# ur-whitelab/nmrgnn

Measured on AMD Instinct MI355X. Metric: atoms/s (fwd+bwd) on 256-atom/16-neighbor synthetic graphs, higher is better.
Workload: dtype f32 (2xf16-piece MFMA, f32 accumulate)

## Files before the change

### include/nmrgnn_hip.h

```cpp
#ifndef NMRGNN_HIP_H
#define NMRGNN_HIP_H

#include <stdint.h>

#ifdef __cplusplus
extern "C" {
#endif

#define NG_ABI_VERSION 9

enum {
  NG_OK = 0,
  NG_ERR_INVALID = -1,
  NG_ERR_HIP = -2,
  NG_ERR_NOMEM = -3,
  NG_ERR_UNSUPPORTED = -4
};

enum { NG_ACT_NONE = 0, NG_ACT_SOFTPLUS = 1, NG_ACT_RELU = 2, NG_ACT_TANH = 3 };

typedef struct ng_ctx ng_ctx;

int ng_abi_version(void);
int ng_ctx_create(int device, ng_ctx** out);
// ... 88 lines not shown

int ng_mp_aggregate(ng_ctx*, void* stream, int64_t N, int K, int F, int E, const float* h,
                    const int32_t* nlist, const float* e, float* A);

int ng_mp_layer_fwd(ng_ctx*, void* stream, int64_t N, int K, int F, int E, int act, int residual,
                    const float* h, const int32_t* nlist, const float* e, const float* inv_degree,
                    const float* w, float* h_out, float* A_save, float* s_save);
int ng_mp_layer_wants_aggregate(int F, int E, int K);

int ng_mp_layer_bwd(ng_ctx*, void* stream, int64_t N, int K, int F, int E, int act,
                    const float* h, const int32_t* nlist, const float* e, const float* inv_degree,
                    const float* w, const float* A_save, const float* s_save,
                    const int32_t* csc_ptr, const int32_t* csc_edge, const float* dh_out,
                    float* dh_in, float* de, int de_accum, float* dw);

int ng_mp_edge_records(ng_ctx*, void* stream, int64_t N, int K, int E, const int32_t* csc_ptr,
                       const int32_t* csc_edge, const float* e, float* rec);
int ng_mp_layer_bwd_rec(ng_ctx*, void* stream, int64_t N, int K, int F, int E, int act,
                    const float* h, const int32_t* nlist, const float* e, const float* inv_degree,
                    const float* w, const float* A_save, const float* s_save,
                    const int32_t* csc_ptr, const int32_t* csc_edge, const float* dh_out,
                    float* dh_in, float* de, int de_accum, float* dw, const float* csc_rec);

int ng_mp_aggregate_csr(ng_ctx*, void* stream, int64_t N, int F, int E, const float* h,
                        const int32_t* row_ptr, const int32_t* col, const float* e, float* A);
int ng_mp_layer_fwd_csr(ng_ctx*, void* stream, int64_t N, int64_t nnz, int F, int E, int act, int residual,
                        const float* h, const int32_t* row_ptr, const int32_t* col, const float* e,
                        const float* inv_degree, const float* w, float* h_out, float* A_save, float* s_save);
int ng_mp_layer_bwd_csr(ng_ctx*, void* stream, int64_t N, int64_t nnz, int F, int E, int act, const float* h,
                        const int32_t* row_ptr, const int32_t* col, const int32_t* row_of, const float* e,
                        const float* inv_degree, const float* w, const float* A_save, const float* s_save,
                        const int32_t* csc_ptr, const int32_t* csc_edge, const float* dh_out, float* dh_in,
                        float* de, int de_accum, float* dw);

int ng_mp_layer_fwd_short(ng_ctx*, void* stream, int64_t N, int K, int F, int E, int act, int residual, const float* h,
                          const int32_t* nlist, const float* e, const float* inv_degree, const float* w, float* h_out);
int ng_mp_layer_fwd_short_csr(ng_ctx*, void* stream, int64_t N, int F, int E, int act, int residual, const float* h,
                              const int32_t* row_ptr, const int32_t* col, const float* e, const float* inv_degree,
                              const float* w, float* h_out);
int ng_mp_layer_short_ok(int64_t N, int K, int F, int E);
int ng_fc_head_ok(int64_t N, int F, int L, int C, int act);
int ng_fc_head_fwd(ng_ctx*, void* stream, int64_t N, int F, int L, int C, int act, const float* x,
                   const float* const* W, const float* const* b, const float* Wout, const float* bout,
                   const float* atoms, const float* pstd, const float* pavg, float* peaks);

int ng_build_incoming_lists(ng_ctx*, void* stream, int64_t N, int K, int64_t n_entries, const int32_t* nlist,
// ... 110 lines not shown
```

### nmrgnn_amd/_lib.py

```python
from __future__ import annotations

import ctypes as C
import os
import threading

_HERE = os.path.dirname(os.path.abspath(__file__))
LIB_PATH = os.environ.get("NMRGNN_HIP_LIB") or os.path.join(_HERE, "csrc", "libnmrgnn_hip.so")

NG_ACT_NONE, NG_ACT_SOFTPLUS, NG_ACT_RELU, NG_ACT_TANH = 0, 1, 2, 3
ACT_CODES = {None: NG_ACT_NONE, "linear": NG_ACT_NONE, "softplus": NG_ACT_SOFTPLUS, "relu": NG_ACT_RELU,
             "tanh": NG_ACT_TANH}

_c_float_p = C.POINTER(C.c_float)
_c_int32_p = C.POINTER(C.c_int32)
_vp = C.c_void_p
_i64 = C.c_int64
_u64 = C.c_uint64
_int = C.c_int
_f = C.c_float

SIGNATURES = {
    "ng_abi_version": (_int, []),
    "ng_ctx_create": (_int, [_int, C.POINTER(_vp)]),
    "ng_ctx_destroy": (None, [_vp]),
# ... 38 lines not shown
                                    C.POINTER(_vp), C.POINTER(_vp), _vp, _vp]),
    "ng_edge_mlp_bwd_live": (_int, [_vp, _vp, _i64, _int, _int, _int, _int, _vp, _vp, _vp, _vp, _vp, _f,
                                    C.POINTER(_vp), _vp, _vp, C.POINTER(_vp), C.POINTER(_vp), _int]),
    "ng_edge_mlp_dinput": (_int, [_vp, _vp, _i64, _int, _int, _int, _int, _vp, _vp, _vp, _vp, _vp, _f,
                                  C.POINTER(_vp), C.POINTER(_vp), _vp, _vp, _vp]),
    "ng_positions_grad": (_int, [_vp, _vp, _i64, _int, _vp, _vp, _vp, _vp, _f, _vp, _vp, _vp]),
    "ng_positions_grad_csr": (_int, [_vp, _vp, _i64, _i64, _vp, _vp, _vp, _vp, _vp, _f, _vp, _vp, _vp]),
    "ng_positions_grad_pbc": (_int, [_vp, _vp, _i64, _int, _vp, _vp, _vp, _vp, _f, _vp, _vp, _int, _vp, _int, _vp]),
    "ng_positions_grad_csr_pbc": (_int, [_vp, _vp, _i64, _i64, _vp, _vp, _vp, _vp, _vp, _f, _vp, _vp, _int, _vp, _int, _vp]),
    "ng_box_grad": (_int, [_vp, _vp, _i64, _int, _vp, _vp, _vp, _vp, _f, _int, _vp, _vp, _int, _vp, _vp]),
    "ng_box_grad_csr": (_int, [_vp, _vp, _i64, _i64, _vp, _vp, _vp, _vp, _f, _int, _vp, _vp, _int, _vp, _vp]),
    "ng_restraint_loss": (_int, [_vp, _vp, _int, _i64, _vp, _vp, _vp, _vp, _vp]),
    "ng_restraint_loss_ex": (_int, [_vp, _vp, _int, _i64, _int, _vp, _vp, _vp, _vp, _vp, _f, _vp, _vp, _vp, _vp]),
    "ng_embed_fwd": (_int, [_vp, _vp, _i64, _int, _int, _vp, _vp, _vp]),
    "ng_embed_bwd": (_int, [_vp, _vp, _i64, _int, _int, _vp, _vp, _vp]),
    "ng_mp_aggregate": (_int, [_vp, _vp, _i64, _int, _int, _int, _vp, _vp, _vp, _vp]),
    "ng_mp_layer_fwd": (_int, [_vp, _vp, _i64, _int, _int, _int, _int, _int, _vp, _vp, _vp, _vp, _vp,
                               _vp, _vp, _vp]),
    "ng_mp_layer_bwd": (_int, [_vp, _vp, _i64, _int, _int, _int, _int, _vp, _vp, _vp, _vp, _vp,
                               _vp, _vp, _vp, _vp, _vp, _vp, _vp, _int, _vp]),
    "ng_mp_layer_bwd_rec": (_int, [_vp, _vp, _i64, _int, _int, _int, _int, _vp, _vp, _vp, _vp, _vp,
                               _vp, _vp, _vp, _vp, _vp, _vp, _vp, _int, _vp, _vp]),
    "ng_mp_edge_records": (_int, [_vp, _vp, _i64, _int, _int, _vp, _vp, _vp, _vp]),
    "ng_mp_aggregate_csr": (_int, [_vp, _vp, _i64, _int, _int, _vp, _vp, _vp, _vp, _vp]),
    "ng_mp_layer_fwd_csr": (_int, [_vp, _vp, _i64, _i64, _int, _int, _int, _int, _vp, _vp, _vp, _vp, _vp, _vp,
                                   _vp, _vp, _vp]),
    "ng_mp_layer_bwd_csr": (_int, [_vp, _vp, _i64, _i64, _int, _int, _int, _vp, _vp, _vp, _vp, _vp, _vp, _vp,
                                   _vp, _vp, _vp, _vp, _vp, _vp, _vp, _int, _vp]),
    "ng_build_incoming_lists": (_int, [_vp, _vp, _i64, _int, _i64, _vp, _vp, _vp, _vp, _vp]),
    "ng_incoming_lists_scratch_bytes": (C.c_size_t, [_i64, _i64]),
    "ng_cutoff_count": (_int, [_vp, _vp, _int, _int, _f, _vp, _vp]),
    "ng_cutoff_fill": (_int, [_vp, _vp, _int, _int, _f, _f, _vp, _vp, _vp, _vp, _vp]),
    "ng_cutoff_fill_rows": (_int, [_vp, _vp, _int, _int, _f, _f, _vp, _vp, _vp, _vp, _vp, _vp]),
    "ng_cutoff_count_pbc": (_int, [_vp, _vp, _int, _int, _f, _vp, _vp, _int, _vp]),
    "ng_cutoff_fill_rows_pbc": (_int, [_vp, _vp, _int, _int, _f, _f, _vp, _vp, _int, _vp, _vp, _vp, _vp, _vp]),
    "ng_exclusive_scan_i32": (_int, [_vp, _vp, _i64, _vp, _vp]),
    "ng_dense_fwd": (_int, [_vp, _vp, _i64, _int, _int, _int, _int, _vp, _vp, _vp, _vp, _vp]),
    "ng_dense_bwd": (_int, [_vp, _vp, _i64, _int, _int, _int, _int, _vp, _vp, _vp, _vp, _vp, _vp,
                            _vp]),
    "ng_head_fwd": (_int, [_vp, _vp, _i64, _int, _int, _vp, _vp, _vp, _vp, _vp, _vp, _vp, _vp]),
    "ng_head_fwd_dropout": (_int, [_vp, _vp, _i64, _int, _int, _vp, _u64, _u64, _f, _vp, _vp, _vp, _vp, _vp, _vp, _vp]),
    "ng_head_bwd": (_int, [_vp, _vp, _i64, _int, _int, _vp, _vp, _vp, _vp, _vp, _vp, _vp, _vp, _vp]),
    "ng_head_loss_blocks": (_int, [_vp, _int, _int, _int, _i64]),
    "ng_head_loss_bwd": (_int, [_vp, _vp, _i64, _int, _int, _int, _i64, _vp, _u64, _u64, _f, _vp, _vp, _vp, _vp, _vp, _vp, _vp,
                               _vp, _vp, _f, _vp, _vp, _vp]),
    "ng_head_loss_reduce": (_int, [_vp, _vp, _vp, _int, _int, _int, _vp, _vp, _vp]),
# ... 128 lines not shown
```

### nmrgnn_amd/csrc/capi.hip

```cpp
#include <cmath>
#include <algorithm>
#include <cstring>
#include <map>
#include <new>

#include "ng_common.h"
#include "ng_internal.h"
#include "reduce.cuh"

namespace ng {

static Switches g_sw;
static bool g_sw_loaded = false;

static bool env_is(const char* name, const char* value) {
  const char* v = getenv(name);
  return v && !strcmp(v, value);
}

static void load_switches() {
  Switches s;
  s.edge_math_fp32 = env_is("NG_EDGE_MATH", "fp32");
  s.edge_bwd_math_fp32 = env_is("NG_EDGE_BWD_MATH", "fp32");
  s.gemm_math_fp32 = env_is("NG_GEMM_MATH", "fp32");
  s.edge_layered = env_is("NG_EDGE_PATH", "layered");
  s.mp_layered = env_is("NG_MP_PATH", "layered");
  s.fc_layered = env_is("NG_FC_PATH", "layered");
  s.dense_generic = env_is("NG_DENSE_PATH", "generic");
  s.head_generic = env_is("NG_HEAD_PATH", "generic");
  s.knn_serial = env_is("NG_KNN", "serial");
  s.knn_lanes = env_is("NG_KNN", "lanes");
  s.knn_cells = env_is("NG_KNN", "cells");
  s.knn_brute = env_is("NG_KNN", "brute");
  s.mp_gg_on = env_is("NG_MP_GG", "1");
  s.mp_gw_nowin = env_is("NG_MP_GW", "nowin");
  s.mp_w16 = !env_is("NG_MP_W16", "0");
  s.mp_wave = env_is("NG_MP_WAVE", "1") ? 1 : (env_is("NG_MP_WAVE", "0") ? 0 : -1);
  s.reduce_narrow = env_is("NG_REDUCE", "narrow");
  if (const char* v = getenv("NG_MP_GG_MIN_ROWS")) { const long long r = atoll(v); if (r >= 1) s.mp_gg_min_rows = r; }
  g_sw = s;
  g_sw_loaded = true;
}

const Switches& sw() {
  if (!g_sw_loaded) load_switches();
  return g_sw;
}

RangeGuard range_guard_begin(ng_ctx* ctx) {
  RangeGuard g;
  char* s = (char*)small_scratch(ctx);
  g.word = s ? reinterpret_cast<unsigned*>(s + NG_SMALL_BYTES - 64) : nullptr;
  if (++ctx->range_epoch == 0) ++ctx->range_epoch;
  g.epoch = ctx->range_epoch;
  return g;
}

const uint64_t* replay_state(ng_ctx* ctx) {
  if (!ctx->replay_armed) return nullptr;
  char* s = (char*)small_scratch(ctx);
// ... 445 lines not shown
```

### nmrgnn_amd/csrc/ng_common.h

```cpp
#pragma once
#include <hip/hip_runtime.h>

#include <cstdint>
#include <cstdio>
#include <string>
#include <map>
#include <utility>
#include <vector>

#include "../../include/nmrgnn_hip.h"

namespace ng {
struct RangeGuard {
  unsigned* word;
  unsigned epoch;
};

enum PackKind : int {
  PK_NONE = 0,
  PK_EDGE_H2 = 1,
  PK_EDGE_WT = 2,
  PK_EDGE_F32 = 3,
  PK_MPW_FWD = 4,
  PK_MPW_BWD = 5,
// ... 44 lines not shown
  uint64_t wjobs_hash = 0;
  std::vector<char> wjobs_host;
  uint32_t range_epoch = 0;
  void* comm = nullptr;
  int comm_rank = 0, comm_world = 1;
  bool defer_reduce = false;
  void* rq = nullptr;
  bool replay_armed = false;
  std::map<uint64_t, void*> wjobs_private;
  std::map<uint64_t, std::vector<WImage*>> wjobs_private_sel;
  uint64_t replay_token = 0;
};

namespace ng {

struct Switches {
  bool edge_math_fp32 = false, edge_bwd_math_fp32 = false, gemm_math_fp32 = false;
  bool edge_layered = false, mp_layered = false, fc_layered = false;
  bool dense_generic = false, head_generic = false, knn_serial = false, knn_cells = false, knn_brute = false;
  bool mp_gg_on = false;
  bool mp_gw_nowin = false;
  int mp_wave = -1;
  bool mp_w16 = true;
  bool reduce_narrow = false;
  bool knn_lanes = false;
  int64_t mp_gg_min_rows = 8192;
};
const Switches& sw();

struct DeviceGuard {
  int prev = -1;
  bool switched = false;
  explicit DeviceGuard(int dev) {
    if (hipGetDevice(&prev) == hipSuccess && prev != dev) switched = hipSetDevice(dev) == hipSuccess;
  }
  ~DeviceGuard() {
    if (switched) (void)hipSetDevice(prev);
  }
};

inline int fail(ng_ctx* ctx, int code, const std::string& msg) {
  if (ctx) ctx->err = msg;
  return code;
}

#define NG_HIP(ctx, expr)                                                              \
// ... 36 lines not shown
```

### nmrgnn_amd/engine.py

```python
from __future__ import annotations

import ctypes as C
import os

import numpy as np
import torch

from . import _lib
from ._lib import ptr, ptr_array
from .graph import GraphBatch
from .params import ParamStore

ACT = {None: 0, "linear": 0, "softplus": 1, "relu": 2, "tanh": 3}
DROPOUT_RATE = 0.2
FUSED_TAIL_MAX_ATOMS = 16384


def rbf_grid(low, high, count):
    lo, hi = np.float32(low), np.float32(high)
    delta = (hi - lo) / np.float32(count - 1)
    c = (lo + delta * np.arange(count, dtype=np.float32)).astype(np.float32)
    c[-1] = hi
    return c, float(np.float32(c[1] - c[0]))


def edge_path(edge_table, use_live_edges, live_kernels, E, n_edges, min_edges, is_csr, capturing):
    fits = n_edges * E * 4 < (1 << 31)
    sized = edge_table and E <= 8 and n_edges >= min_edges and fits
    if live_kernels and fits:
        return "table" if sized else ("live" if use_live_edges else "slots")
    if sized and not is_csr and not capturing:
        return "table_host"
    return "slots"


class Tape:
    __slots__ = ("batch", "d_eff", "z_save", "z_layout", "e", "h", "A", "S", "fx", "g", "drop_mask",
                 "peaks", "edge_path", "live", "table", "loss", "dpeaks", "dg", "head_partial")


class Engine:
    _ids = 0

    def __init__(self, hp, num_elem, peak_std=None, peak_avg=None, device=None, seed=1234):
        if not torch.cuda.is_available():
            raise _lib.NGError("nmrgnn_amd needs an AMD GPU (torch.cuda.is_available() is False); "
                               "there is no CPU fallback")
        if device is None:
            device = torch.device("cuda", torch.cuda.current_device())
        self.device = torch.device(device)
        if self.device.index is None:
            self.device = torch.device("cuda", torch.cuda.current_device())
        self.ctx = _lib.get_context(self.device.index)
        self.lib = self.ctx.lib
        self.hp = hp
        self.C = int(num_elem)
        self.F = hp.get('atom_feature_size')
        self.E = hp.get('edge_feature_size')
        self.H = hp.get('edge_hidden_size')
        self.L = hp.get('mp_layers')
        self.Le = hp.get('edge_fc_layers')
# ... 103 lines not shown
                self._ck(lib.ng_add_noise_live(h, st, seed, 0, ne, ptr(batch.edges), ptr(None if noise is None else noise.reshape(-1)),
                                               self.sigma, ptr(pos), ptr(d_eff)), "ng_add_noise_live")
        elif training and self.sigma > 0:
            d_eff = self._new(ne)
            if noise is None:
                self._ck(lib.ng_add_noise(h, st, seed, 0, ne, ptr(d_src), self.sigma, ptr(d_eff)), "ng_add_noise")
            else:
                noise = noise.reshape(-1)
                self._ck(lib.ng_add_scaled(h, st, ne, ptr(d_src), ptr(noise), self.sigma, ptr(d_eff)),
                         "ng_add_scaled")
        table = self._edge_table_build(batch, live, d_eff, tape, training) if path in ("table", "table_host") else None
        if path == "table_host" and table is None:
            path = "slots"
        if path == "table":
            rows = table["gate"][1:]
        e = self._new(ne, E)
        z_save, z_layout = None, 0
        if path != "table_host":
            z_save, z_layout = self._edge_mlp_fwd(ne, d_src, d_eff, e, tape, perm, rows)
        if table is not None:
            self._ck(lib.ng_edge_table_interp(h, st, ne, E, table["T"], ptr(batch.edges), ptr(d_eff), ptr(pos),
                                              ptr(table["rng"]), ptr(table["e_all"]), ptr(table["gate"]), ptr(e)),
                     "ng_edge_table_interp")
        h0 = self._new(N, F)
        self._ck(lib.ng_embed_fwd(h, st, N, self.C, F, ptr(batch.atoms), ptr(P["embed/kernel"]),
                                  ptr(h0)), "ng_embed_fwd")
        hs, As, Ss = [h0], [], []
        for l in range(self.L):
            hn = self._new(N, F)
            S = self._new(N, F) if (tape and self.mp_act != 0) else None
            if batch.is_csr and not tape and N <= FUSED_TAIL_MAX_ATOMS and lib.ng_mp_layer_short_ok(N, 1, F, E):
                A = None
                self._ck(lib.ng_mp_layer_fwd_short_csr(h, st, N, F, E, self.mp_act, 1, ptr(hs[-1]), ptr(batch.row_ptr),
                                                       ptr(batch.nlist), ptr(e), ptr(batch.inv_degree), ptr(P[f"mp/{l}/w"]),
                                                       ptr(hn)), "ng_mp_layer_fwd_short_csr")
            elif batch.is_csr:
                A = self._new(N, E, F) if tape else None
                self._ck(lib.ng_mp_layer_fwd_csr(h, st, N, ne, F, E, self.mp_act, 1, ptr(hs[-1]),
                                                 ptr(batch.row_ptr), ptr(batch.nlist), ptr(e),
                                                 ptr(batch.inv_degree), ptr(P[f"mp/{l}/w"]), ptr(hn), ptr(A),
                                                 ptr(S)), "ng_mp_layer_fwd_csr")
            elif not tape and N <= FUSED_TAIL_MAX_ATOMS and lib.ng_mp_layer_short_ok(N, K, F, E):
                A = None
                self._ck(lib.ng_mp_layer_fwd_short(h, st, N, K, F, E, self.mp_act, 1, ptr(hs[-1]), ptr(batch.nlist_c), ptr(e),
                                                   ptr(batch.inv_degree), ptr(P[f"mp/{l}/w"]), ptr(hn)), "ng_mp_layer_fwd_short")
            else:
                A = self._new(N, E, F) if (tape and lib.ng_mp_layer_wants_aggregate(F, E, K)) else None
                self._ck(lib.ng_mp_layer_fwd(h, st, N, K, F, E, self.mp_act, 1, ptr(hs[-1]),
                                             ptr(batch.nlist_c), ptr(e), ptr(batch.inv_degree),
                                             ptr(P[f"mp/{l}/w"]), ptr(hn), ptr(A), ptr(S)),
                         "ng_mp_layer_fwd")
            hs.append(hn)
            As.append(A)
            Ss.append(S)
# ... 32 lines not shown
        elif training and self.use_dropout and dropout_mask is None:
            mask = self._new(N, Fh)
            self._ck(lib.ng_head_fwd_dropout(h, st, N, Fh, self.C, ptr(g), seed, 1 << 40, 1.0 - DROPOUT_RATE, ptr(mask),
                                             ptr(P["out/kernel"]), ptr(P["out/bias"]), ptr(batch.atoms),
                                             ptr(self.peak_std), ptr(self.peak_avg), ptr(peaks)), "ng_head_fwd_dropout")
        else:
            if training and self.use_dropout:
                mask = dropout_mask.reshape(N, Fh).contiguous()
            self._ck(lib.ng_head_fwd(h, st, N, Fh, self.C, ptr(g), ptr(mask), ptr(P["out/kernel"]),
                                     ptr(P["out/bias"]), ptr(batch.atoms), ptr(self.peak_std),
                                     ptr(self.peak_avg), ptr(peaks)), "ng_head_fwd")
        if loss is not None and nb == 0:
            y, w, gw = loss
            loss_t, dpeaks = self.loss_l2(batch, y, w, peaks)
            if gw != 1.0:
                dpeaks.mul_(gw)
        if tape:
            tp = Tape()
            tp.loss, tp.dpeaks, tp.dg, tp.head_partial = loss_t, dpeaks, dg, head_partial
            tp.batch, tp.d_eff, tp.z_save, tp.e = batch, d_eff, z_save, e
            tp.z_layout = z_layout
            tp.edge_path, tp.live, tp.table = path, live, table
            tp.h, tp.A, tp.S, tp.fx, tp.g, tp.drop_mask, tp.peaks = hs, As, Ss, fx, g, mask, peaks
            self.tape = tp
        return peaks

    EDGE_TABLE_POINTS = 4096

    def _table_points(self):
        return self.EDGE_TABLE_POINTS if self.E <= 4 else self.EDGE_TABLE_POINTS // 2

    def _edge_weights(self):
        P = self.params
        return [P[f"edge_fc/{t}/kernel"] for t in range(self.Le)], [P[f"edge_fc/{t}/bias"] for t in range(self.Le)]

    def _edge_grads(self, view=None):
        view = view or self.params.g
        return [view(f"edge_fc/{t}/kernel") for t in range(self.Le)], [view(f"edge_fc/{t}/bias") for t in range(self.Le)]

    def _edge_mlp_fwd(self, n, d_src, d_eff, e, tape, perm=None, rows=None):
        lib, h, st = self.lib, self.ctx.handle, self._st()
        z, z_layout = None, 0
        if tape:
            z = self._new(self.Le - 1, n, self.H)
            z_layout = int(lib.ng_edge_tape_layout(self.H, self.E, self.Le, self.fc_act, n))
        W, B = self._edge_weights()
# ... 120 lines not shown
            dpeaks = dpeaks.contiguous()
            dg = self._new(N, Fh)
            self._ck(lib.ng_head_bwd(h, st, N, Fh, self.C, ptr(tp.g), ptr(tp.drop_mask),
                                     ptr(P["out/kernel"]), ptr(b.atoms), ptr(self.peak_std),
                                     ptr(dpeaks), ptr(dg), ptr(wg("out/kernel")), ptr(wg("out/bias"))),
                     "ng_head_bwd")
        dx = self._new(N, F)
        Wfc = [P[f"fc/{t}/kernel"] for t in range(self.Lf)]
        ns = int(lib.ng_fc_block_scratch_floats(N, F, self.Lf))
        scratch = self._new(ns) if ns else None
        self._ck(lib.ng_fc_block_bwd(h, st, N, F, self.Lf, self.fc_act, ptr_array(tp.fx), ptr(tp.g),
                                     ptr_array(Wfc), ptr(dg), ptr(dx),
                                     warr([wg(f"fc/{t}/kernel") for t in range(self.Lf)]),
                                     warr([wg(f"fc/{t}/bias") for t in range(self.Lf)]),
                                     ptr(scratch)), "ng_fc_block_bwd")
        csc_ptr, csc_edge = b.csc()
        de = self._new(ne, E)
        rec = None
        if E <= 3 and not b.is_csr:
            rec = self._new(ne, 4)
            self._ck(lib.ng_mp_edge_records(h, st, N, K, E, ptr(csc_ptr), ptr(csc_edge), ptr(tp.e), ptr(rec)),
                     "ng_mp_edge_records")
        dh = dx
        for l in reversed(range(self.L)):
            dhn = self._new(N, F)
            if b.is_csr:
                self._ck(lib.ng_mp_layer_bwd_csr(h, st, N, ne, F, E, self.mp_act, ptr(tp.h[l]), ptr(b.row_ptr),
                                                 ptr(b.nlist), ptr(b.row_of), ptr(tp.e), ptr(b.inv_degree),
                                                 ptr(P[f"mp/{l}/w"]), ptr(tp.A[l]), ptr(tp.S[l]), ptr(csc_ptr),
                                                 ptr(csc_edge), ptr(dh), ptr(dhn), ptr(de),
                                                 0 if l == self.L - 1 else 1, ptr(wg(f"mp/{l}/w"))),
                         "ng_mp_layer_bwd_csr")
                dh = dhn
                continue
            self._ck(lib.ng_mp_layer_bwd_rec(h, st, N, K, F, E, self.mp_act, ptr(tp.h[l]), ptr(b.nlist_c),
                                         ptr(tp.e), ptr(b.inv_degree), ptr(P[f"mp/{l}/w"]),
                                         ptr(tp.A[l]), ptr(tp.S[l]), ptr(csc_ptr), ptr(csc_edge),
                                         ptr(dh), ptr(dhn), ptr(de), 0 if l == self.L - 1 else 1,
                                         ptr(wg(f"mp/{l}/w")), ptr(rec)), "ng_mp_layer_bwd")
            dh = dhn
        if not param_grad:
            self._edge_dinput(tp, de, edge_grad)
            self.tape = None
            return
        self._ck(lib.ng_embed_bwd(h, st, N, self.C, F, ptr(b.atoms), ptr(dh),
                                  ptr(P.g("embed/kernel"))), "ng_embed_bwd")
        self._ck(lib.ng_flush_reductions(h, st), "ng_flush_reductions")
        if on_node_grads is not None:
            on_node_grads()
        if tp.edge_path == "slots":
            self._edge_mlp_bwd(ne, b.edges, tp.d_eff, tp.z_save, tp.z_layout, de, self._edge_grads())
        elif tp.edge_path == "live":
            perm, _, d_c, n_live = tp.live
            self._edge_mlp_bwd(ne, d_c, tp.d_eff, tp.z_save, tp.z_layout, de, self._edge_grads(), perm, n_live)
        elif tp.edge_path == "table_host":
            self._edge_table_backward(tp, de, self._edge_grads())
        else:
            names = [f"edge_fc/{t}/{k}" for t in range(self.Le) for k in ("kernel", "bias")]
            o0 = min(P.offsets[n] for n in names)
            o1 = max(P.offsets[n] + int(np.prod(P.shapes[n])) for n in names)
            tmp = self._new(o1 - o0)
            tv = lambda n: tmp[P.offsets[n] - o0:P.offsets[n] - o0 + int(np.prod(P.shapes[n]))]
            perm, _, d_c, _ = tp.live
            self._edge_mlp_bwd(ne, d_c, tp.d_eff, tp.z_save, tp.z_layout, de, self._edge_grads(tv), perm, tp.table["gate"][1:])
            self._edge_table_backward(tp, de, self._edge_grads())
            blk = P.grad[o0:o1]
            self._ck(lib.ng_add_scaled(h, st, o1 - o0, ptr(blk), ptr(tmp), 1.0, ptr(blk)), "ng_add_scaled")
        if edge_grad is not None:
            self._edge_dinput(tp, de, edge_grad)
        self.tape = None
# ... 47 lines not shown
```

Before: 43.70 million.

## Fuse embedding into first message-passing layer via precomputed Wemb·W product

Adds a specialised layer-0 path that exploits the one-hot/low-dimensional atom embedding. It folds the embedding matrix into the layer weights (M = Wemb·W) and aggregates neighbour atom features times edge features (T, size C·E) instead of gathering F-wide hidden states. The backward pass uses the saved T and dM partials and recovers the dw and dWemb gradients in a finish kernel. This removes the separate embed forward/backward and the wide layer-0 gather, at the cost of extra prep and finish kernels, new saved buffers and a narrower shape envelope (C·E ≤ 64, F a multiple of 64 up to 256).

```diff
diff --git a/include/nmrgnn_hip.h b/include/nmrgnn_hip.h
--- a/include/nmrgnn_hip.h
+++ b/include/nmrgnn_hip.h
@@ -134,6 +134,19 @@
                     const int32_t* csc_ptr, const int32_t* csc_edge, const float* dh_out,
                     float* dh_in, float* de, int de_accum, float* dw, const float* csc_rec);
 
+int ng_mp_layer0_ok(int64_t N, int K, int F, int E, int C);
+int ng_mp_layer0_enabled(void);
+int ng_mp_layer0_fwd(ng_ctx*, void* stream, int64_t N, int K, int F, int E, int C, int act, int residual,
+                     const float* atoms, const float* Wemb, const int32_t* nlist, const float* e,
+                     const float* inv_degree, const float* w, const float* h0, float* h_out, float* s_save,
+                     float* T_save);
+int ng_mp_layer0_bwd(ng_ctx*, void* stream, int64_t N, int K, int F, int E, int C, int act, int residual,
+                     const float* atoms, const float* Wemb, const int32_t* nlist, const float* inv_degree,
+                     const float* w, const float* s_save, const float* T_save, const float* dh_out, float* de,
+                     int de_accum, float* dM);
+int ng_mp_layer0_finish(ng_ctx*, void* stream, int F, int E, int C, int residual, const float* Wemb, const float* w,
+                        const float* dM, float* dw, float* dWemb);
+
 int ng_mp_aggregate_csr(ng_ctx*, void* stream, int64_t N, int F, int E, const float* h,
                         const int32_t* row_ptr, const int32_t* col, const float* e, float* A);
 int ng_mp_layer_fwd_csr(ng_ctx*, void* stream, int64_t N, int64_t nnz, int F, int E, int act, int residual,
diff --git a/nmrgnn_amd/_lib.py b/nmrgnn_amd/_lib.py
--- a/nmrgnn_amd/_lib.py
+++ b/nmrgnn_amd/_lib.py
@@ -84,6 +84,11 @@
     "ng_mp_layer_bwd_rec": (_int, [_vp, _vp, _i64, _int, _int, _int, _int, _vp, _vp, _vp, _vp, _vp,
                                _vp, _vp, _vp, _vp, _vp, _vp, _vp, _int, _vp, _vp]),
     "ng_mp_edge_records": (_int, [_vp, _vp, _i64, _int, _int, _vp, _vp, _vp, _vp]),
+    "ng_mp_layer0_ok": (_int, [_i64, _int, _int, _int, _int]),
+    "ng_mp_layer0_enabled": (_int, []),
+    "ng_mp_layer0_fwd": (_int, [_vp, _vp, _i64, _int, _int, _int, _int, _int, _int] + [_vp] * 10),
+    "ng_mp_layer0_bwd": (_int, [_vp, _vp, _i64, _int, _int, _int, _int, _int, _int] + [_vp] * 9 + [_int, _vp]),
+    "ng_mp_layer0_finish": (_int, [_vp, _vp, _int, _int, _int, _int, _vp, _vp, _vp, _vp, _vp]),
     "ng_mp_aggregate_csr": (_int, [_vp, _vp, _i64, _int, _int, _vp, _vp, _vp, _vp, _vp]),
     "ng_mp_layer_fwd_csr": (_int, [_vp, _vp, _i64, _i64, _int, _int, _int, _int, _vp, _vp, _vp, _vp, _vp, _vp,
                                    _vp, _vp, _vp]),
diff --git a/nmrgnn_amd/csrc/capi.hip b/nmrgnn_amd/csrc/capi.hip
--- a/nmrgnn_amd/csrc/capi.hip
+++ b/nmrgnn_amd/csrc/capi.hip
@@ -36,6 +36,7 @@
   s.mp_gw_nowin = env_is("NG_MP_GW", "nowin");
   s.mp_w16 = !env_is("NG_MP_W16", "0");
   s.mp_wave = env_is("NG_MP_WAVE", "1") ? 1 : (env_is("NG_MP_WAVE", "0") ? 0 : -1);
+  s.mp_l0 = !env_is("NG_MP_L0", "0");
   s.reduce_narrow = env_is("NG_REDUCE", "narrow");
   if (const char* v = getenv("NG_MP_GG_MIN_ROWS")) { const long long r = atoll(v); if (r >= 1) s.mp_gg_min_rows = r; }
   g_sw = s;
diff --git a/nmrgnn_amd/csrc/mp_layer0.hip b/nmrgnn_amd/csrc/mp_layer0.hip
--- /dev/null
+++ b/nmrgnn_amd/csrc/mp_layer0.hip
@@ -0,0 +1,444 @@
+#include "mp_win_common.cuh"
+#include "ng_internal.h"
+#include "reduce.cuh"
+
+namespace ng {
+namespace l0 {
+
+constexpr int TA = 64;
+constexpr int NT = 256;
+constexpr int FC = 64;
+constexpr int LDP = FC + 4;
+constexpr int WG_PER_CU = 2;
+
+inline int round_up(int v, int m) { return (v + m - 1) / m * m; }
+inline int grid_for(const ng_ctx* ctx, int64_t ntiles) {
+  return (int)std::min<int64_t>(ntiles, (int64_t)WG_PER_CU * std::max(ctx->num_cu, 1));
+}
+
+static hipError_t allow_lds(const ng_ctx* ctx, const void* fn, size_t lds) {
+  static std::map<std::pair<const void*, int>, size_t> granted;
+  if (lds <= 64 * 1024) return hipSuccess;
+  size_t& have = granted[std::make_pair(fn, ctx->device)];
+  if (lds <= have) return hipSuccess;
+  const hipError_t e = hipFuncSetAttribute(fn, hipFuncAttributeMaxDynamicSharedMemorySize, (int)lds);
+  if (e == hipSuccess) have = lds;
+  return e;
+}
+
+__device__ __forceinline__ int64_t clamp_row(int idx, int64_t N) {
+  return idx < 0 ? 0 : (idx >= N ? N - 1 : (int64_t)idx);
+}
+
+__global__ __launch_bounds__(256) void mp_l0_prep_kernel(int F, int E, int CE, const float* __restrict__ emb,
+                                                         const float* __restrict__ w, float* __restrict__ M) {
+  const int idx = blockIdx.x * 256 + threadIdx.x;
+  if (idx >= CE * F) return;
+  const int j = idx / F, m = idx - j * F;
+  const int c = j / E, n = j - c * E;
+  float s = 0.f;
+  for (int l = 0; l < F; ++l) s = fmaf(emb[c * F + l], w[((int64_t)l * F + m) * E + n], s);
+  M[idx] = s;
+}
+
+struct FwdArgs {
+  int64_t N, ntiles;
+  int K, F, E, C, CE, CEp, Cp, act, residual;
+  const float *atoms, *emb, *e, *inv, *M, *h0;
+  const int32_t* nlist;
+  float *h_out, *s_save, *T_save;
+};
+
+__global__ __launch_bounds__(NT) void mp_l0_fwd_kernel(FwdArgs a) {
+  extern __shared__ __attribute__((aligned(16))) float sm[];
+  const int CEp = a.CEp, Cp = a.Cp, CE = a.CE, C = a.C, E = a.E, K = a.K, F = a.F;
+  const bool recompute = a.residual && !a.h0;
+  float* Ts = sm;
+  float* Ms = Ts + TA * CEp;
+  float* invs = Ms + CEp * FC;
+  float* Xs = invs + TA;
+  float* Es = Xs + TA * Cp;
+  const int t = threadIdx.x, m = t & 63, g = t >> 6;
+  const int nch = F / FC;
+  for (int p = t; p < TA * CEp; p += NT) Ts[p] = 0.f;
+  for (int p = t; p < CEp * FC; p += NT) Ms[p] = 0.f;
+  if (recompute) {
+    for (int p = t; p < TA * Cp; p += NT) Xs[p] = 0.f;
+    for (int p = t; p < Cp * FC; p += NT) Es[p] = 0.f;
+  }
+  __syncthreads();
+  if (nch == 1) {
+    for (int p = t; p < CE * FC; p += NT) Ms[p] = a.M[p];
+    if (recompute)
+      for (int p = t; p < C * FC; p += NT) Es[p] = a.emb[p];
+  }
+  for (int64_t tile = blockIdx.x; tile < a.ntiles; tile += gridDim.x) {
+    const int64_t i0 = tile * TA;
+    __syncthreads();
+    for (int p = t; p < TA * CE; p += NT) {
+      const int at = p / CE, j = p - at * CE;
+      const int c = j / E, n = j - c * E;
+      const int64_t i = i0 + at;
+      float s = 0.f;
+      if (i < a.N) {
+        const int32_t* nl = a.nlist + i * K;
+        const float* ee = a.e + i * K * E + n;
+#pragma unroll 4
+        for (int k = 0; k < K; ++k) s = fmaf(ee[k * E], a.atoms[clamp_row(nl[k], a.N) * C + c], s);
+        if (a.T_save) a.T_save[i * CE + j] = s;
+      }
+      Ts[at * CEp + j] = s;
+    }
+    if (t < TA) invs[t] = i0 + t < a.N ? a.inv[i0 + t] : 0.f;
+    if (recompute)
+      for (int p = t; p < TA * C; p += NT) {
+        const int at = p / C, c = p - at * C;
+        Xs[at * Cp + c] = i0 + at < a.N ? a.atoms[(i0 + at) * C + c] : 0.f;
+      }
+    for (int fc = 0; fc < nch; ++fc) {
+      if (nch > 1) {
+        __syncthreads();
+        for (int p = t; p < CE * FC; p += NT) Ms[p] = a.M[(p / FC) * F + fc * FC + (p % FC)];
+        if (recompute)
+          for (int p = t; p < C * FC; p += NT) Es[p] = a.emb[(p / FC) * F + fc * FC + (p % FC)];
+      }
+      __syncthreads();
+      float acc[16], res[16];
+#pragma unroll
+      for (int r = 0; r < 16; ++r) { acc[r] = 0.f; res[r] = 0.f; }
+      for (int j4 = 0; j4 < CEp; j4 += 4) {
+        const float m0 = Ms[(j4 + 0) * FC + m], m1 = Ms[(j4 + 1) * FC + m], m2 = Ms[(j4 + 2) * FC + m], m3 = Ms[(j4 + 3) * FC + m];
+#pragma unroll
+        for (int r = 0; r < 16; ++r) {
+          const float4 tv = *reinterpret_cast<const float4*>(Ts + (g * 16 + r) * CEp + j4);
+          acc[r] = fmaf(tv.w, m3, fmaf(tv.z, m2, fmaf(tv.y, m1, fmaf(tv.x, m0, acc[r]))));
+        }
+      }
+      if (recompute)
+        for (int c4 = 0; c4 < Cp; c4 += 4) {
+          const float m0 = Es[(c4 + 0) * FC + m], m1 = Es[(c4 + 1) * FC + m], m2 = Es[(c4 + 2) * FC + m], m3 = Es[(c4 + 3) * FC + m];
+#pragma unroll
+          for (int r = 0; r < 16; ++r) {
+            const float4 xv = *reinterpret_cast<const float4*>(Xs + (g * 16 + r) * Cp + c4);
+            res[r] = fmaf(xv.w, m3, fmaf(xv.z, m2, fmaf(xv.y, m1, fmaf(xv.x, m0, res[r]))));
+          }
+        }
+#pragma unroll
+      for (int r = 0; r < 16; ++r) {
+        const int64_t i = i0 + g * 16 + r;
+        if (i < a.N) {
+          const int64_t o = i * F + fc * FC + m;
+          const float v = act_apply(a.act, invs[g * 16 + r] * acc[r]);
+          if (a.s_save) a.s_save[o] = v;
+          a.h_out[o] = a.residual ? v + (a.h0 ? a.h0[o] : res[r]) : v;
+        }
+      }
+    }
+  }
+}
+
+struct BwdArgs {
+  int64_t N, ntiles;
+  int K, F, E, C, CE, CEp, Cp, GJ, act, residual, de_accum;
+  const float *atoms, *inv, *M, *s_save, *T_save, *dh_out;
+  const int32_t* nlist;
+  float *de, *part_m, *part_x;
+};
+
+template <int NCH, bool DW>
+__global__ __launch_bounds__(NT) void mp_l0_bwd_kernel(BwdArgs a) {
+  extern __shared__ __attribute__((aligned(16))) float sm[];
+  const int CEp = a.CEp, Cp = a.Cp, CE = a.CE, C = a.C, E = a.E, K = a.K, F = a.F, GJ = a.GJ, GP = a.GJ + 1;
+  const bool resid = DW && a.residual;
+  float* dPs = sm;
+  float* Ms = dPs + TA * LDP;
+  float* Gs = Ms + GJ * LDP;
+  float* invs = Gs + TA * GP;
+  float* Ts = invs + TA;
+  float* dHs = Ts + TA * CEp;
+  float* Xs = dHs + TA * LDP;
+  const int t = threadIdx.x, m = t & 63, g = t >> 6;
+  const int ag = t & 15, jg = t >> 4;
+  const int ny = GJ / 16;
+  const int q4 = CEp / 4, x4 = Cp / 4;
+  float macc[NCH][16], xacc[NCH][16];
+#pragma unroll
+  for (int f = 0; f < NCH; ++f)
+#pragma unroll
+    for (int u = 0; u < 16; ++u) { macc[f][u] = 0.f; xacc[f][u] = 0.f; }
+  for (int p = t; p < GJ * LDP; p += NT) Ms[p] = 0.f;
+  if (DW) {
+    for (int p = t; p < TA * CEp; p += NT) Ts[p] = 0.f;
+    if (resid)
+      for (int p = t; p < TA * Cp; p += NT) Xs[p] = 0.f;
+  }
+  __syncthreads();
+  if (NCH == 1)
+    for (int p = t; p < CE * FC; p += NT) Ms[(p / FC) * LDP + (p % FC)] = a.M[p];
+  for (int64_t tile = blockIdx.x; tile < a.ntiles; tile += gridDim.x) {
+    const int64_t i0 = tile * TA;
+    __syncthreads();
+    if (t < TA) invs[t] = i0 + t < a.N ? a.inv[i0 + t] : 0.f;
+    if (DW) {
+      for (int p = t; p < TA * CE; p += NT) {
+        const int at = p / CE, j = p - at * CE;
+        Ts[at * CEp + (j & 3) * q4 + (j >> 2)] = i0 + at < a.N ? a.T_save[(i0 + at) * CE + j] : 0.f;
+      }
+      if (resid)
+        for (int p = t; p < TA * C; p += NT) {
+          const int at = p / C, c = p - at * C;
+          Xs[at * Cp + (c & 3) * x4 + (c >> 2)] = i0 + at < a.N ? a.atoms[(i0 + at) * C + c] : 0.f;
+        }
+    }
+    float gacc[4][4];
+#pragma unroll
+    for (int x = 0; x < 4; ++x)
+#pragma unroll
+      for (int y = 0; y < 4; ++y) gacc[x][y] = 0.f;
+#pragma unroll
+    for (int fc = 0; fc < NCH; ++fc) {
+      __syncthreads();
+#pragma unroll
+      for (int r = 0; r < 4; ++r) {
+        const int at = (t >> 4) + 16 * r, c4 = (t & 15) * 4;
+        const int64_t i = i0 + at;
+        float4 d = f4zero(), dh = f4zero();
+        if (i < a.N) {
+          const int64_t o = i * F + fc * FC + c4;
+          dh = *reinterpret_cast<const float4*>(a.dh_out + o);
+          d = dh;
+          if (a.act != NG_ACT_NONE) {
+            const float4 s = *reinterpret_cast<const float4*>(a.s_save + o);
+            d.x *= act_grad_from_out(a.act, s.x); d.y *= act_grad_from_out(a.act, s.y);
+            d.z *= act_grad_from_out(a.act, s.z); d.w *= act_grad_from_out(a.act, s.w);
+          }
+          const float sc = invs[at];
+          d.x *= sc; d.y *= sc; d.z *= sc; d.w *= sc;
+        }
+        *reinterpret_cast<float4*>(dPs + at * LDP + c4) = d;
+        if (resid) *reinterpret_cast<float4*>(dHs + at * LDP + c4) = dh;
+      }
+      if (NCH > 1)
+        for (int p = t; p < CE * FC; p += NT) Ms[(p / FC) * LDP + (p % FC)] = a.M[(p / FC) * F + fc * FC + (p % FC)];
+      __syncthreads();
+      for (int c4 = 0; c4 < FC; c4 += 4) {
+        float4 dv[4];
+#pragma unroll
+        for (int x = 0; x < 4; ++x) dv[x] = *reinterpret_cast<const float4*>(dPs + (ag + 16 * x) * LDP + c4);
+#pragma unroll
+        for (int y = 0; y < 4; ++y)
+          if (y < ny) {
+            const float4 mv = *reinterpret_cast<const float4*>(Ms + (jg + 16 * y) * LDP + c4);
+#pragma unroll
+            for (int x = 0; x < 4; ++x)
+              gacc[x][y] = fmaf(dv[x].w, mv.w, fmaf(dv[x].z, mv.z, fmaf(dv[x].y, mv.y, fmaf(dv[x].x, mv.x, gacc[x][y]))));
+          }
+      }
+      if (DW) {
+        for (int at = 0; at < TA; ++at) {
+          const float dp = dPs[at * LDP + m];
+#pragma unroll
+          for (int u4 = 0; u4 < 4; ++u4)
+            if (u4 * 16 < CEp) {
+              const float4 tv = *reinterpret_cast<const float4*>(Ts + at * CEp + g * q4 + u4 * 4);
+              macc[fc][u4 * 4 + 0] = fmaf(tv.x, dp, macc[fc][u4 * 4 + 0]);
+              macc[fc][u4 * 4 + 1] = fmaf(tv.y, dp, macc[fc][u4 * 4 + 1]);
+              macc[fc][u4 * 4 + 2] = fmaf(tv.z, dp, macc[fc][u4 * 4 + 2]);
+              macc[fc][u4 * 4 + 3] = fmaf(tv.w, dp, macc[fc][u4 * 4 + 3]);
+            }
+          if (resid) {
+            const float dh = dHs[at * LDP + m];
+#pragma unroll
+            for (int u4 = 0; u4 < 4; ++u4)
+              if (u4 * 16 < Cp) {
+                const float4 xv = *reinterpret_cast<const float4*>(Xs + at * Cp + g * x4 + u4 * 4);
+                xacc[fc][u4 * 4 + 0] = fmaf(xv.x, dh, xacc[fc][u4 * 4 + 0]);
+                xacc[fc][u4 * 4 + 1] = fmaf(xv.y, dh, xacc[fc][u4 * 4 + 1]);
+                xacc[fc][u4 * 4 + 2] = fmaf(xv.z, dh, xacc[fc][u4 * 4 + 2]);
+                xacc[fc][u4 * 4 + 3] = fmaf(xv.w, dh, xacc[fc][u4 * 4 + 3]);
+              }
+          }
+        }
+      }
+    }
+#pragma unroll
+    for (int x = 0; x < 4; ++x)
+#pragma unroll
+      for (int y = 0; y < 4; ++y)
+        if (y < ny) Gs[(ag + 16 * x) * GP + jg + 16 * y] = gacc[x][y];
+    __syncthreads();
+    const int KE = K * E;
+    for (int p = t; p < TA * KE; p += NT) {
+      const int at = p / KE, rem = p - at * KE;
+      const int k = rem / E, n = rem - k * E;
+      const int64_t i = i0 + at;
+      if (i < a.N) {
+        const float* x = a.atoms + clamp_row(a.nlist[i * K + k], a.N) * C;
+        const float* gr = Gs + at * GP + n;
+        float s = 0.f;
+#pragma unroll 4
+        for (int c = 0; c < C; ++c) s = fmaf(x[c], gr[c * E], s);
+        const int64_t o = i * KE + rem;
+        a.de[o] = a.de_accum ? a.de[o] + s : s;
+      }
+    }
+  }
+  if (DW) {
+    float* pm = a.part_m + (int64_t)blockIdx.x * CE * F;
+#pragma unroll
+    for (int fc = 0; fc < NCH; ++fc)
+#pragma unroll
+      for (int u = 0; u < 16; ++u)
+        if (g + 4 * u < CE) pm[(int64_t)(g + 4 * u) * F + fc * FC + m] = macc[fc][u];
+    if (resid) {
+      float* px = a.part_x + (int64_t)blockIdx.x * C * F;
+#pragma unroll
+      for (int fc = 0; fc < NCH; ++fc)
+#pragma unroll
+        for (int u = 0; u < 16; ++u)
+          if (g + 4 * u < C) px[(int64_t)(g + 4 * u) * F + fc * FC + m] = xacc[fc][u];
+    }
+  }
+}
+
+__global__ __launch_bounds__(256) void mp_l0_finish_kernel(int F, int E, int C, int residual, const float* __restrict__ emb,
+                                                           const float* __restrict__ w, const float* __restrict__ dM,
+                                                           const float* __restrict__ dXH, float* __restrict__ dw,
+                                                           float* __restrict__ demb) {
+  const int64_t idx = (int64_t)blockIdx.x * 256 + threadIdx.x;
+  const int64_t nw = (int64_t)F * F * E;
+  if (idx < nw) {
+    const int l = (int)(idx / (F * E)), rem = (int)(idx - (int64_t)l * F * E);
+    const int m = rem / E, n = rem - m * E;
+    float s = 0.f;
+    for (int c = 0; c < C; ++c) s = fmaf(emb[c * F + l], dM[(int64_t)(c * E + n) * F + m], s);
+    dw[idx] = s;
+  } else if (idx < nw + (int64_t)C * F) {
+    const int o = (int)(idx - nw);
+    const int c = o / F, l = o - c * F;
+    float s = residual ? dXH[o] : 0.f;
+    for (int n = 0; n < E; ++n)
+      for (int m = 0; m < F; ++m) s = fmaf(dM[(int64_t)(c * E + n) * F + m], w[((int64_t)l * F + m) * E + n], s);
+    demb[o] = s;
+  }
+}
+
+static bool shape_ok(int K, int F, int E, int C) {
+  return K >= 1 && E >= 1 && C >= 1 && C * E <= 64 && F >= 64 && F % 64 == 0 && F <= 256;
+}
+
+}
+}
+
+using namespace ng;
+using namespace ng::l0;
+
+extern "C" int ng_mp_layer0_ok(int64_t N, int K, int F, int E, int C) { return N >= 0 && shape_ok(K, F, E, C) ? 1 : 0; }
+
+extern "C" int ng_mp_layer0_enabled(void) { return sw().mp_l0 && !sw().mp_layered ? 1 : 0; }
+
+extern "C" int ng_mp_layer0_fwd(ng_ctx* ctx, void* stream, int64_t N, int K, int F, int E, int C, int act, int residual,
+                                const float* atoms, const float* Wemb, const int32_t* nlist, const float* e,
+                                const float* inv_degree, const float* w, const float* h0, float* h_out, float* s_save,
+                                float* T_save) {
+  if (!ctx) return NG_ERR_INVALID;
+  hipStream_t st = (hipStream_t)stream;
+  NG_REQUIRE(ctx, shape_ok(K, F, E, C), "mp_layer0: C*E <= 64, F % 64 == 0, F <= 256");
+  NG_REQUIRE(ctx, N >= 0 && N * (int64_t)std::max(K * E, F) < ((int64_t)1 << 40), "mp_layer0: N");
+  if (N == 0) return NG_OK;
+  NG_REQUIRE(ctx, atoms && Wemb && nlist && e && inv_degree && w && h_out, "mp_layer0_fwd: arguments");
+  const int CE = C * E;
+  float* M = (float*)workspace(ctx, (size_t)CE * F * 4);
+  if (!M) return NG_ERR_NOMEM;
+  ProfScope ps(ctx, st, "mp_l0_fwd");
+  hipLaunchKernelGGL(mp_l0_prep_kernel, dim3((unsigned)cdiv((int64_t)CE * F, 256)), dim3(256), 0, st, F, E, CE, Wemb, w, M);
+  FwdArgs a{};
+  a.N = N; a.ntiles = cdiv(N, TA);
+  a.K = K; a.F = F; a.E = E; a.C = C; a.CE = CE; a.CEp = round_up(CE, 4); a.Cp = round_up(C, 4);
+  a.act = act; a.residual = residual;
+  a.atoms = atoms; a.emb = Wemb; a.e = e; a.inv = inv_degree; a.M = M; a.h0 = h0; a.nlist = nlist;
+  a.h_out = h_out; a.s_save = s_save; a.T_save = T_save;
+  size_t lds = (size_t)(TA * a.CEp + a.CEp * FC + TA) * 4;
+  if (residual && !h0) lds += (size_t)(TA * a.Cp + a.Cp * FC) * 4;
+  NG_HIP(ctx, allow_lds(ctx, (const void*)mp_l0_fwd_kernel, lds));
+  hipLaunchKernelGGL(mp_l0_fwd_kernel, dim3((unsigned)grid_for(ctx, a.ntiles)), dim3(NT), lds, st, a);
+  NG_HIP(ctx, hipGetLastError());
+  return NG_OK;
+}
+
+template <int NCH, bool DW>
+static hipError_t launch_bwd_as(const ng_ctx* ctx, hipStream_t st, int grid, size_t lds, const BwdArgs& a) {
+  const hipError_t e = allow_lds(ctx, (const void*)mp_l0_bwd_kernel<NCH, DW>, lds);
+  if (e != hipSuccess) return e;
+  hipLaunchKernelGGL((mp_l0_bwd_kernel<NCH, DW>), dim3((unsigned)grid), dim3(NT), lds, st, a);
+  return hipGetLastError();
+}
+template <int NCH>
+static hipError_t launch_bwd(const ng_ctx* ctx, hipStream_t st, int grid, size_t lds, bool dw, const BwdArgs& a) {
+  return dw ? launch_bwd_as<NCH, true>(ctx, st, grid, lds, a) : launch_bwd_as<NCH, false>(ctx, st, grid, lds, a);
+}
+
+extern "C" int ng_mp_layer0_bwd(ng_ctx* ctx, void* stream, int64_t N, int K, int F, int E, int C, int act, int residual,
+                                const float* atoms, const float* Wemb, const int32_t* nlist, const float* inv_degree,
+                                const float* w, const float* s_save, const float* T_save, const float* dh_out, float* de,
+                                int de_accum, float* dM) {
+  if (!ctx) return NG_ERR_INVALID;
+  hipStream_t st = (hipStream_t)stream;
+  NG_REQUIRE(ctx, shape_ok(K, F, E, C), "mp_layer0: C*E <= 64, F % 64 == 0, F <= 256");
+  NG_REQUIRE(ctx, N >= 0 && N * (int64_t)std::max(K * E, F) < ((int64_t)1 << 40), "mp_layer0: N");
+  NG_REQUIRE(ctx, act == NG_ACT_NONE || s_save, "mp_layer0_bwd: s_save required for an activation");
+  NG_REQUIRE(ctx, !dM || T_save, "mp_layer0_bwd: the weight gradients need the forward's T");
+  const int CE = C * E;
+  const int64_t n_m = (int64_t)CE * F, n_x = residual ? (int64_t)C * F : 0;
+  if (N == 0) {
+    if (dM) NG_HIP(ctx, hipMemsetAsync(dM, 0, (size_t)(n_m + (int64_t)C * F) * 4, st));
+    return NG_OK;
+  }
+  NG_REQUIRE(ctx, atoms && Wemb && nlist && inv_degree && w && dh_out && de, "mp_layer0_bwd: arguments");
+  BwdArgs a{};
+  a.N = N; a.ntiles = cdiv(N, TA);
+  const int grid = grid_for(ctx, a.ntiles);
+  const size_t m_floats = ((size_t)n_m + 63) / 64 * 64;
+  float* part = nullptr;
+  bool arena = false;
+  if (dM) {
+    part = deferred_partials(ctx, (size_t)grid * (n_m + n_x));
+    arena = part != nullptr;
+  }
+  float* M = (float*)workspace(ctx, (m_floats + (dM && !arena ? (size_t)grid * (n_m + n_x) : 0)) * 4);
+  if (!M) return NG_ERR_NOMEM;
+  if (dM && !arena) part = M + m_floats;
+  ProfScope ps(ctx, st, "mp_l0_bwd");
+  hipLaunchKernelGGL(mp_l0_prep_kernel, dim3((unsigned)cdiv(n_m, 256)), dim3(256), 0, st, F, E, CE, Wemb, w, M);
+  a.K = K; a.F = F; a.E = E; a.C = C; a.CE = CE; a.CEp = round_up(CE, 16); a.Cp = round_up(C, 16); a.GJ = round_up(CE, 16);
+  a.act = act; a.residual = residual; a.de_accum = de_accum;
+  a.atoms = atoms; a.inv = inv_degree; a.M = M; a.s_save = s_save; a.T_save = T_save; a.dh_out = dh_out; a.nlist = nlist;
+  a.de = de; a.part_m = part; a.part_x = part && residual ? part + (int64_t)grid * n_m : nullptr;
+  size_t lds = (size_t)(TA * LDP + a.GJ * LDP + TA * (a.GJ + 1) + TA) * 4;
+  if (dM) lds += (size_t)(TA * a.CEp) * 4 + (residual ? (size_t)(TA * LDP + TA * a.Cp) * 4 : 0);
+  switch (F / FC) {
+    case 1: NG_HIP(ctx, launch_bwd<1>(ctx, st, grid, lds, dM != nullptr, a)); break;
+    case 2: NG_HIP(ctx, launch_bwd<2>(ctx, st, grid, lds, dM != nullptr, a)); break;
+    case 3: NG_HIP(ctx, launch_bwd<3>(ctx, st, grid, lds, dM != nullptr, a)); break;
+    default: NG_HIP(ctx, launch_bwd<4>(ctx, st, grid, lds, dM != nullptr, a)); break;
+  }
+  if (!dM) return NG_OK;
+  int rc = reduce_or_defer(ctx, st, part, grid, n_m, dM);
+  if (rc) return rc;
+  if (residual) rc = reduce_or_defer(ctx, st, a.part_x, grid, n_x, dM + n_m);
+  return rc;
+}
+
+extern "C" int ng_mp_layer0_finish(ng_ctx* ctx, void* stream, int F, int E, int C, int residual, const float* Wemb,
+                                   const float* w, const float* dM, float* dw, float* dWemb) {
+  if (!ctx) return NG_ERR_INVALID;
+  hipStream_t st = (hipStream_t)stream;
+  NG_REQUIRE(ctx, shape_ok(1, F, E, C), "mp_layer0: C*E <= 64, F % 64 == 0, F <= 256");
+  NG_REQUIRE(ctx, Wemb && w && dM && dw && dWemb, "mp_layer0_finish: arguments");
+  ProfScope ps(ctx, st, "mp_l0_finish");
+  const int64_t items = (int64_t)F * F * E + (int64_t)C * F;
+  hipLaunchKernelGGL(mp_l0_finish_kernel, dim3((unsigned)cdiv(items, 256)), dim3(256), 0, st, F, E, C, residual, Wemb, w, dM,
+                     dM + (int64_t)C * E * F, dw, dWemb);
+  NG_HIP(ctx, hipGetLastError());
+  return NG_OK;
+}
diff --git a/nmrgnn_amd/csrc/ng_common.h b/nmrgnn_amd/csrc/ng_common.h
--- a/nmrgnn_amd/csrc/ng_common.h
+++ b/nmrgnn_amd/csrc/ng_common.h
@@ -90,6 +90,7 @@
   bool mp_gw_nowin = false;
   int mp_wave = -1;
   bool mp_w16 = true;
+  bool mp_l0 = true;
   bool reduce_narrow = false;
   bool knn_lanes = false;
   int64_t mp_gg_min_rows = 8192;
diff --git a/nmrgnn_amd/engine.py b/nmrgnn_amd/engine.py
--- a/nmrgnn_amd/engine.py
+++ b/nmrgnn_amd/engine.py
@@ -36,7 +36,7 @@
 
 class Tape:
     __slots__ = ("batch", "d_eff", "z_save", "z_layout", "e", "h", "A", "S", "fx", "g", "drop_mask",
-                 "peaks", "edge_path", "live", "table", "loss", "dpeaks", "dg", "head_partial")
+                 "peaks", "edge_path", "live", "table", "loss", "dpeaks", "dg", "head_partial", "T0")
 
 
 class Engine:
@@ -186,14 +186,25 @@
             self._ck(lib.ng_edge_table_interp(h, st, ne, E, table["T"], ptr(batch.edges), ptr(d_eff), ptr(pos),
                                               ptr(table["rng"]), ptr(table["e_all"]), ptr(table["gate"]), ptr(e)),
                      "ng_edge_table_interp")
-        h0 = self._new(N, F)
-        self._ck(lib.ng_embed_fwd(h, st, N, self.C, F, ptr(batch.atoms), ptr(P["embed/kernel"]),
-                                  ptr(h0)), "ng_embed_fwd")
+        short = not tape and N <= FUSED_TAIL_MAX_ATOMS and bool(lib.ng_mp_layer_short_ok(N, K, F, E))
+        use_l0 = self.L > 0 and not batch.is_csr and not short and bool(lib.ng_mp_layer0_enabled()) \
+            and bool(lib.ng_mp_layer0_ok(N, K, F, E, self.C))
+        h0 = T0 = None
+        if not use_l0:
+            h0 = self._new(N, F)
+            self._ck(lib.ng_embed_fwd(h, st, N, self.C, F, ptr(batch.atoms), ptr(P["embed/kernel"]),
+                                      ptr(h0)), "ng_embed_fwd")
         hs, As, Ss = [h0], [], []
         for l in range(self.L):
             hn = self._new(N, F)
             S = self._new(N, F) if (tape and self.mp_act != 0) else None
-            if batch.is_csr and not tape and N <= FUSED_TAIL_MAX_ATOMS and lib.ng_mp_layer_short_ok(N, 1, F, E):
+            if l == 0 and use_l0:
+                A = None
+                T0 = self._new(N, self.C * E) if tape else None
+                self._ck(lib.ng_mp_layer0_fwd(h, st, N, K, F, E, self.C, self.mp_act, 1, ptr(batch.atoms),
+                                              ptr(P["embed/kernel"]), ptr(batch.nlist_c), ptr(e), ptr(batch.inv_degree),
+                                              ptr(P["mp/0/w"]), None, ptr(hn), ptr(S), ptr(T0)), "ng_mp_layer0_fwd")
+            elif batch.is_csr and not tape and N <= FUSED_TAIL_MAX_ATOMS and lib.ng_mp_layer_short_ok(N, 1, F, E):
                 A = None
                 self._ck(lib.ng_mp_layer_fwd_short_csr(h, st, N, F, E, self.mp_act, 1, ptr(hs[-1]), ptr(batch.row_ptr),
                                                        ptr(batch.nlist), ptr(e), ptr(batch.inv_degree), ptr(P[f"mp/{l}/w"]),
@@ -272,6 +283,7 @@
             tp.z_layout = z_layout
             tp.edge_path, tp.live, tp.table = path, live, table
             tp.h, tp.A, tp.S, tp.fx, tp.g, tp.drop_mask, tp.peaks = hs, As, Ss, fx, g, mask, peaks
+            tp.T0 = T0
             self.tape = tp
         return peaks
 
@@ -438,7 +450,14 @@
             self._ck(lib.ng_mp_edge_records(h, st, N, K, E, ptr(csc_ptr), ptr(csc_edge), ptr(tp.e), ptr(rec)),
                      "ng_mp_edge_records")
         dh = dx
+        dM0 = None
         for l in reversed(range(self.L)):
+            if l == 0 and tp.T0 is not None:
+                dM0 = self._new((self.C * E + self.C) * F) if param_grad else None
+                self._ck(lib.ng_mp_layer0_bwd(h, st, N, K, F, E, self.C, self.mp_act, 1, ptr(b.atoms), ptr(P["embed/kernel"]),
+                                              ptr(b.nlist_c), ptr(b.inv_degree), ptr(P["mp/0/w"]), ptr(tp.S[0]), ptr(tp.T0),
+                                              ptr(dh), ptr(de), 0 if self.L == 1 else 1, ptr(dM0)), "ng_mp_layer0_bwd")
+                continue
             dhn = self._new(N, F)
             if b.is_csr:
                 self._ck(lib.ng_mp_layer_bwd_csr(h, st, N, ne, F, E, self.mp_act, ptr(tp.h[l]), ptr(b.row_ptr),
@@ -459,9 +478,13 @@
             self._edge_dinput(tp, de, edge_grad)
             self.tape = None
             return
-        self._ck(lib.ng_embed_bwd(h, st, N, self.C, F, ptr(b.atoms), ptr(dh),
-                                  ptr(P.g("embed/kernel"))), "ng_embed_bwd")
+        if dM0 is None:
+            self._ck(lib.ng_embed_bwd(h, st, N, self.C, F, ptr(b.atoms), ptr(dh),
+                                      ptr(P.g("embed/kernel"))), "ng_embed_bwd")
         self._ck(lib.ng_flush_reductions(h, st), "ng_flush_reductions")
+        if dM0 is not None:
+            self._ck(lib.ng_mp_layer0_finish(h, st, F, E, self.C, 1, ptr(P["embed/kernel"]), ptr(P["mp/0/w"]), ptr(dM0),
+                                             ptr(P.g("mp/0/w")), ptr(P.g("embed/kernel"))), "ng_mp_layer0_finish")
         if on_node_grads is not None:
             on_node_grads()
         if tp.edge_path == "slots":
```

New measurement: 41.26 million. 5.6% lower.
